# ethz-asl/laser_slam

Measured on AMD Instinct MI355X. Metric: scans_per_sec, higher is better.
Workload: dtype f32

## Files before the change

### laser_slam_amd/csrc/lsgpu_cone.hip.h

```cpp
#pragma once
#include "lsgpu_knn.hip.h"

namespace lsgpu {

constexpr int kConeGF4 = 3;
constexpr int kConePad = 16;
constexpr uint32_t kConeMaxWin = 512;

struct ConeDev {
  float ox, oy, oz;
  float z0, rs;
  float cs;
  int rows, cols;
  const float4* soa;
  const uint32_t* map;
  const uint32_t* tab;
  const float4* rowz;
};

__device__ __forceinline__ void cone_dir(float vx, float vy, float vz, float& inv_rho, float& zeta, float& pa, float& rxy,
                                         float& inv_h) {
  const float r2 = __fmaf_rn(vy, vy, vx * vx);
  inv_rho = __builtin_amdgcn_rsqf(__fmaf_rn(vz, vz, r2));
  rxy = __builtin_amdgcn_sqrtf(r2);
// ... 119 lines not shown
      const float4 X1 = p1[0], Y1 = p1[1], Z1 = p1[2];
      const f32x2 d0 = dist2_pair(q2x, q2y, q2z, f32x2{X.x, X.y}, f32x2{Y.x, Y.y}, f32x2{Z.x, Z.y});
      const f32x2 d1 = dist2_pair(q2x, q2y, q2z, f32x2{X.z, X.w}, f32x2{Y.z, Y.w}, f32x2{Z.z, Z.w});
      const f32x2 e0 = dist2_pair(q2x, q2y, q2z, f32x2{X1.x, X1.y}, f32x2{Y1.x, Y1.y}, f32x2{Z1.x, Z1.y});
      const f32x2 e1 = dist2_pair(q2x, q2y, q2z, f32x2{X1.z, X1.w}, f32x2{Y1.z, Y1.w}, f32x2{Z1.z, Z1.w});
      const float m4 = fminf(fminf(fminf(d0.x, d0.y), d1.x), d1.y);
      const float n4 = fminf(fminf(fminf(e0.x, e0.y), e1.x), e1.y);
      sec = __builtin_amdgcn_fmed3f(best, m4, sec);
      best = fminf(best, m4);
      sec = __builtin_amdgcn_fmed3f(best, n4, sec);
      best = fminf(best, n4);
    }
  }
}

#ifndef LSGPU_CONE_WAVES
#define LSGPU_CONE_WAVES 4
#endif
#ifndef LSGPU_CONE_OCC
#define LSGPU_CONE_OCC 8
#endif
constexpr int kConeRowSlots = 4;

struct ConeRec { float qx, qy, qz, ub, lbn; int id_in, j; uint32_t pad; };

__device__ __forceinline__ void cone_barrier_lds() {
  asm volatile("s_waitcnt lgkmcnt(0)\n\ts_barrier" ::: "memory");
}
__device__ __forceinline__ uint32_t wave_min_u32(uint32_t v) { return ~wave_max_u32(~v); }

template <int WAVES, bool PROBE = false>
__global__ __launch_bounds__(WAVES * 64, LSGPU_CONE_OCC) void k_knn_cone(KnnArgs a, ConeDev c) {
  __shared__ ConeRec rec[WAVES * 64];
  __shared__ unsigned long long ne_mask[16];
  __shared__ uint32_t wcount[WAVES], wbelow[WAVES];
  extern __shared__ float4 rowz_sh[];
  const int lane = threadIdx.x & 63, w = threadIdx.x >> 6;
#ifdef LSGPU_KNN_STATS
  const long long ts0 = clock64();
  const uint32_t wall0 = (uint32_t)wall_clock64();
  long long t_rows = 0, t_stage = 0, t_eval = 0;
  uint32_t n_chunks = 0, n_steps = 0, n_groups = 0, n_rowslots = 0;
#endif
  const uint32_t tile = blockIdx.x * (uint32_t)WAVES + (uint32_t)w;
  int j = (int)(tile * 64u) + lane;
  const bool act = j < a.nq;
  float4 rraw = make_float4(0.f, 0.f, 0.f, 0.f), mp = rraw;
// ... 60 lines not shown
  if (sel_on) {
    const uint32_t bits = __float_as_uint(ub);
    const unsigned long long below = __ballot(act && skip && bits < sel_lo);
    if (act && skip && bits >= sel_lo && bits - sel_lo < sel_span) sel_inside(bits);
    nbelow1 = (uint32_t)__popcll(below);
  }
#ifdef LSGPU_KNN_STATS
  const long long ts2 = clock64();
#endif
  const unsigned long long sm = __ballot(act && !skip);
  if (lane == 0) { wcount[w] = (uint32_t)__popcll(sm); wbelow[w] = nbelow1; }
  cone_barrier_lds();
  uint32_t before = 0, total = 0;
#pragma unroll
  for (int k = 0; k < WAVES; ++k) { const uint32_t n = wcount[k]; before += k < w ? n : 0u; total += n; }
  if (sel_on && threadIdx.x == 0) {
    uint32_t nb = 0u;
#pragma unroll
    for (int k = 0; k < WAVES; ++k) nb += wbelow[k];
    if (nb) atomicAdd(&a.sel_below[(blockIdx.x & (kSelBelowSlots - 1)) * kSelBelowStride], nb);
  }
  if (act && !skip) {
    ConeRec r;
    r.qx = qx; r.qy = qy; r.qz = qz; r.ub = ub; r.lbn = lbn; r.id_in = id_in; r.j = j; r.pad = 0u;
    const uint32_t at = before + (uint32_t)__popcll(sm & ((1ull << lane) - 1ull));
    rec[at] = r;
  }
  cone_barrier_lds();
#ifdef LSGPU_KNN_STATS
  const long long ts3 = clock64();
  if (lane == 0 && dbg) {
    dbg[0] = (uint32_t)(ts1 - ts0); dbg[1] = (uint32_t)(ts2 - ts1); dbg[2] = (uint32_t)(ts3 - ts2);
    dbg[3] = 1u; dbg[10] = (uint32_t)(ts3 - ts0); dbg[11] = wall0; dbg[12] = (uint32_t)wall_clock64();
    dbg[13] = (uint32_t)__popcll(sm);
  }
#endif
  if ((uint32_t)(w * 64) >= total) return;
  const bool ing = (uint32_t)(w * 64 + lane) < total;
  {
    const ConeRec r = rec[w * 64 + lane];
    qx = r.qx; qy = r.qy; qz = r.qz; ub = r.ub; lbn = r.lbn; id_in = r.id_in; j = r.j;
  }
  float inv_rho, zeta, pa, rxy, inv_h;
  cone_dir(qx - c.ox, qy - c.oy, qz - c.oz, inv_rho, zeta, pa, rxy, inv_h);
  float ubs = ub;
  if (PROBE) {
    const bool pr = ing && fabsf(zeta) <= 1.5f && pa >= 0.f && pa <= 4.f;
    const int rq = (int)cone_clampu(floorf((zeta - c.z0) * c.rs), c.rows - 1);
    const int cq = (int)cone_clampu(floorf(pa * c.cs), c.cols - 1);
    const uint32_t p_first = (uint32_t)__builtin_amdgcn_readfirstlane((int)wave_max_u32(pr ? ~(uint32_t)max(rq - 2, 0) : 0u));
    const uint32_t p_last = wave_max_u32(pr ? (uint32_t)min(rq + 2, c.rows - 1) + 1u : 0u);
    float pb = INFINITY, ps = INFINITY;
    for (uint32_t row = ~p_first; row < p_last; ++row) {
      const float4 rz = rowz_sh[row];
      if (!(rz.x <= rz.y)) continue;
      const bool in = pr && (int)row >= rq - 2 && (int)row <= rq + 2;
      const uint32_t base = row * (uint32_t)c.cols;
      uint32_t st_ = 0u, en_ = 0u;
      if (in) {
        st_ = c.tab[base + (uint32_t)max(cq - 1, 0)];
        en_ = c.tab[base + (uint32_t)min(cq + 1, c.cols - 1) + 1u];
      }
      const uint32_t g0 = st_ >> 2;
      const uint32_t len = en_ > st_ ? min(((en_ + 3u) >> 2) - g0, 4u) : 0u;
      cone_eval_window(c, g0, len, qx, qy, qz, pb, ps);
    }
    ubs = fminf(ub, pb);
  }
  const float lim0 = prune_lim(ubs, gap, cap2s);
  const float R = __builtin_amdgcn_sqrtf(lim0) * (1.0f + 1e-5f) + 1e-7f;
  bool fb = false;
  float best = INFINITY, sec = INFINITY, bs4 = INFINITY;
  float4 bpt = make_float4(0.f, 0.f, 0.f, 0.f);
  bool found = false;
  uint32_t bgrp = 0xFFFFFFFFu;
  {
    const float s = R * inv_rho * (1.0f + 1e-5f) + 4e-6f;
    const float ce = rxy * inv_rho;
    bool cone = ing && s <= 0.5f && ce > 0.f && ce <= 1.5f;
    const float alpha = s * (1.0f + 0.2f * s * s) + 2e-6f;
    const float alpha2 = alpha * alpha;
    const float dz = __fmaf_rn(ce, s, fabsf(zeta) * s * s) + 2e-6f;
    const float gq = (rxy * inv_h) * (rxy * inv_h) * (1.0f + 1e-6f);
    const float inv_ce = __builtin_amdgcn_rcpf(ce) * (1.0f + 1e-6f);
    const uint32_t r_lo = cone_clampu(floorf((zeta - dz - c.z0) * c.rs), c.rows - 1);
    const uint32_t r_hi = cone_clampu(floorf((zeta + dz - c.z0) * c.rs), c.rows - 1);
    fb = ing && !cone;
    const int cols = c.cols;
    const f32x2 q2x = {qx, qx}, q2y = {qy, qy}, q2z = {qz, qz};
    uint32_t row = (uint32_t)__builtin_amdgcn_readfirstlane((int)wave_min_u32(cone ? r_lo : 0xFFFFFFFFu));
    const uint32_t row_last = wave_max_u32(cone ? r_hi + 1u : 0u);
    int pass = 0;
    uint32_t n_st = 0u, n_en = 0u;
// ... 67 lines not shown
          const float4* __restrict__ p0 = c.soa + (uint32_t)kConeGF4 * (size_t)t;
          const float4* __restrict__ p1 = two ? p0 + kConeGF4 : p0;
          const float4 X = p0[0], Y = p0[1], Z = p0[2];
          const float4 X1 = p1[0], Y1 = p1[1], Z1 = p1[2];
          const f32x2 d0 = dist2_pair(q2x, q2y, q2z, f32x2{X.x, X.y}, f32x2{Y.x, Y.y}, f32x2{Z.x, Z.y});
          const f32x2 d1 = dist2_pair(q2x, q2y, q2z, f32x2{X.z, X.w}, f32x2{Y.z, Y.w}, f32x2{Z.z, Z.w});
          const f32x2 e0 = dist2_pair(q2x, q2y, q2z, f32x2{X1.x, X1.y}, f32x2{Y1.x, Y1.y}, f32x2{Z1.x, Z1.y});
          const f32x2 e1 = dist2_pair(q2x, q2y, q2z, f32x2{X1.z, X1.w}, f32x2{Y1.z, Y1.w}, f32x2{Z1.z, Z1.w});
          const float m4 = fminf(fminf(fminf(d0.x, d0.y), d1.x), d1.y);
          const float n4 = two ? fminf(fminf(fminf(e0.x, e0.y), e1.x), e1.y) : INFINITY;
          sec = __builtin_amdgcn_fmed3f(best, m4, sec);
          bgrp = m4 < best ? t : bgrp;
          best = fminf(best, m4);
          sec = __builtin_amdgcn_fmed3f(best, n4, sec);
          bgrp = n4 < best ? t + 1u : bgrp;
          best = fminf(best, n4);
        }
      }
#ifdef LSGPU_KNN_STATS
      t_eval += clock64() - t_s1;
#endif
    }
  }
  if (bgrp != 0xFFFFFFFFu) {
    const float4* __restrict__ p = c.soa + (uint32_t)kConeGF4 * (size_t)bgrp;
    const float4 X = p[0], Y = p[1], Z = p[2];
    const uint4 m = reinterpret_cast<const uint4*>(c.map)[bgrp];
    const float4 M = make_float4(__uint_as_float(m.x), __uint_as_float(m.y), __uint_as_float(m.z), __uint_as_float(m.w));
    const float e0 = dist2(qx - X.x, qy - Y.x, qz - Z.x), e1 = dist2(qx - X.y, qy - Y.y, qz - Z.y);
    const float e2 = dist2(qx - X.z, qy - Y.z, qz - Z.z), e3 = dist2(qx - X.w, qy - Y.w, qz - Z.w);
    if (e3 == best) bpt = make_float4(X.w, Y.w, Z.w, M.w);
    if (e2 == best) bpt = make_float4(X.z, Y.z, Z.z, M.z);
    if (e1 == best) bpt = make_float4(X.y, Y.y, Z.y, M.y);
    if (e0 == best) bpt = make_float4(X.x, Y.x, Z.x, M.x);
    bs4 = fminf(fmaxf(fminf(e0, e1), fminf(e2, e3)), fminf(fmaxf(e0, e1), fmaxf(e2, e3)));
    found = true;
  }
#ifdef LSGPU_KNN_STATS
  const long long ts5 = clock64();
#endif
  int bi = id_in;
  mp = make_float4(0.f, 0.f, 0.f, __int_as_float(id_in));
  const unsigned long long fbm = __ballot(fb);
  if (fbm) {
    if (fb) {
      best = ub;
      lane_ball_search(a, cap2s, qx, qy, qz, best, bi);
      if (bi != id_in) { const float4 p = a.pts[bi]; mp = make_float4(p.x, p.y, p.z, __int_as_float(bi)); }
    }
    if (lane == 0) atomicAdd(a.strag_count, (uint32_t)__popcll(fbm));
  }
  if (ing) {
    float nb;
    if (fb) {
      nb = best <= cap2s ? sqrtf(best) * (1.0f - 1e-6f) : fmaxf(lbn, sqrtf(cap2s) * (1.0f - 1e-5f));
    } else if (found && best <= ub) {
      mp = bpt;
      sec = fminf(sec, bs4);
      float others = fminf(sec, lim0);
      bool same = __float_as_int(mp.w) == id_in;
      if (sec == best || (!same && best == ub)) {
        mp = canonical_tie(a, qx, qy, qz, best, mp);
        same = __float_as_int(mp.w) == id_in;
      }
      if (!same) others = fminf(others, ub);
      nb = __builtin_amdgcn_sqrtf(others) * (1.0f - 1e-5f);
      if (same) nb = fmaxf(nb, lbn);
    } else {
      nb = fmaxf(__builtin_amdgcn_sqrtf(fminf(best, lim0)) * (1.0f - 1e-5f), lbn);
      best = ub;
    }
    if (a.write_all || __float_as_int(mp.w) != id_in) {
      a.ids[j] = __float_as_int(mp.w);
      a.prev[j] = mp;
    }
    a.d2[j] = best;
    a.lb[j] = nb;
  }
  if (sel_on) {
    const uint32_t bits = __float_as_uint(best);
    const unsigned long long below = __ballot(ing && bits < sel_lo);
    if (ing && bits >= sel_lo && bits - sel_lo < sel_span) sel_inside(bits);
    if (lane == 0 && below) atomicAdd(&a.sel_below[((tile + 32u) & (kSelBelowSlots - 1)) * kSelBelowStride], (uint32_t)__popcll(below));
  }
#ifdef LSGPU_KNN_STATS
  {
    const long long ts9 = clock64();
// ... 12 lines not shown
```

### laser_slam_amd/csrc/lsgpu_knn.hip.h

```cpp
#pragma once
#include "lsgpu_common.hip.h"

namespace lsgpu {

constexpr float kPruneShrink = 1.0f - 2e-6f;
constexpr float kCapSearchMargin2 = 1.05f * 1.05f;
constexpr float kPadCoord = 3e18f;

constexpr int kPriceSlots = 64, kPriceStride = 32;
struct ConePrice {
  float ox, oy, oz, rs, cs, dens4;
  float heavy;
  uint32_t* count;
};
__device__ __forceinline__ float cone_price(const ConePrice& c, float qx, float qy, float qz, float R) {
  const float vx = qx - c.ox, vy = qy - c.oy, vz = qz - c.oz;
  const float r2 = __fmaf_rn(vy, vy, vx * vx);
  const float inv_rho = __builtin_amdgcn_rsqf(__fmaf_rn(vz, vz, r2));
  const float rxy = __builtin_amdgcn_sqrtf(r2);
  const float sn = R * inv_rho, ce = rxy * inv_rho, zeta = fabsf(vz * inv_rho);
  const float g = rxy * __builtin_amdgcn_rcpf(fabsf(vx) + fabsf(vy));
  const float rows = 2.f * (ce * sn + zeta * sn * sn) * c.rs + 1.f;
  const float cols = 2.f * (g * g) * sn * __builtin_amdgcn_rcpf(ce) * c.cs + 1.f;
  const bool served = sn <= 0.5f && ce > 0.05f && ce <= 1.5f;
// ... 92 lines not shown
      continue;
    const uint32_t p0 = a.chunks[cs].start;
    const ChunkDesc dl = a.chunks[l == 0 ? ce - 1 : cs];
    uint32_t p1 = dl.start + dl.count;
    if (p1 - p0 > 256u) p1 = p0 + 256u;
    float best = INFINITY;
    for (uint32_t t = p0; t < p1; t += 4) {
      const float4 c0 = a.pts[t], c1 = a.pts[t + 1], c2 = a.pts[t + 2], c3 = a.pts[t + 3];
      const float d0 = dist2(q.x - c0.x, q.y - c0.y, q.z - c0.z), d1 = dist2(q.x - c1.x, q.y - c1.y, q.z - c1.z);
      const float d2 = dist2(q.x - c2.x, q.y - c2.y, q.z - c2.z), d3 = dist2(q.x - c3.x, q.y - c3.y, q.z - c3.z);
      if (d0 < best) { best = d0; bi = (int)t; bp = c0; }
      if (d1 < best) { best = d1; bi = (int)t + 1; bp = c1; }
      if (d2 < best) { best = d2; bi = (int)t + 2; bp = c2; }
      if (d3 < best) { best = d3; bi = (int)t + 3; bp = c3; }
    }
    bd = best;
    break;
  }
  a.prev[j] = make_float4(bp.x, bp.y, bp.z, __int_as_float(bi));
  a.d2[j] = bd;
  if (a.lb) a.lb[j] = 0.f;
}

__device__ __forceinline__ void lane_ball_search(const KnnArgs& a, float cap2, float qx, float qy, float qz,
                                                 float& best, int& bi) {
  const GridDev& g = a.g;
  float prune = fminf(best, cap2);
  const float R = sqrtf(prune) * (1.0f + 1e-5f) + 1e-7f + kFineSlack * g.hf;
  const int lim = (1 << (g.bits + g.fine)) - 1;
  const int flx = fine_coord(qx - R, g.ox, g.inv_hf, lim), fhx = fine_coord(qx + R, g.ox, g.inv_hf, lim);
  const int fly = fine_coord(qy - R, g.oy, g.inv_hf, lim), fhy = fine_coord(qy + R, g.oy, g.inv_hf, lim);
  const int flz = fine_coord(qz - R, g.oz, g.inv_hf, lim), fhz = fine_coord(qz + R, g.oz, g.inv_hf, lim);
  int l = 0, sh = g.fine;
  for (; l < g.bits; ++l, ++sh)
    if ((fhx >> sh) - (flx >> sh) < 2 && (fhy >> sh) - (fly >> sh) < 2 && (fhz >> sh) - (flz >> sh) < 2)
      break;
  sh = g.fine + l;
  const int x0 = flx >> sh, y0 = fly >> sh, z0 = flz >> sh;
  const int x1 = fhx >> sh, y1 = fhy >> sh, z1 = fhz >> sh;
  const uint32_t mask = g.mask[l];
  const uint4* tab = reinterpret_cast<const uint4*>(g.tab[l]);
  uint4 en[8];
  uint32_t slot[8];
  bool want[8];
#pragma unroll
  for (int c = 0; c < 8; ++c) {
    const int cx = x0 + (c & 1), cy = y0 + ((c >> 1) & 1), cz = z0 + (c >> 2);
    want[c] = cx <= x1 && cy <= y1 && cz <= z1;
    slot[c] = cell_hash((uint32_t)cx, (uint32_t)cy, (uint32_t)cz) & mask;
    en[c] = make_uint4(kEmpty, 0u, 0u, 0u);
    if (want[c]) en[c] = tab[slot[c]];
  }
#pragma unroll
  for (int c = 0; c < 8; ++c) {
    if (!want[c]) continue;
    const uint32_t cx = (uint32_t)(x0 + (c & 1)), cy = (uint32_t)(y0 + ((c >> 1) & 1)), cz = (uint32_t)(z0 + (c >> 2));
    const uint32_t xy = cx | (cy << 16);
    uint4 e = en[c];
    uint32_t sl = slot[c];
    while (!(((e.x ^ xy) | (e.y ^ cz)) == 0u) && e.x != kEmpty) {
      sl = (sl + 1) & mask;
      e = tab[sl];
    }
    if (e.x == kEmpty) continue;
    for (uint32_t ch = e.z; ch < e.w; ++ch) {
      if ((ch & (uint32_t)(kChunkGroup - 1)) == 0u && ch + (uint32_t)kChunkGroup <= e.w) {
        const float4* gd = reinterpret_cast<const float4*>(a.cgroups + ch / (uint32_t)kChunkGroup);
        const float4 g0 = gd[0], g1 = gd[1];
        if (!(box_dist2(g0.x, g0.y, g0.z, g1.x, g1.y, g1.z, qx, qy, qz) * kPruneShrink <= prune)) { ch += (uint32_t)kChunkGroup - 1u; continue; }
      }
      const float4* cd = reinterpret_cast<const float4*>(a.chunks + ch);
      const float4 b0 = cd[0], b1 = cd[1];
      if (!(box_dist2(b0.x, b0.y, b0.z, b1.x, b1.y, b1.z, qx, qy, qz) * kPruneShrink <= prune)) continue;
      const uint32_t st = __float_as_uint(b0.w), cnt = __float_as_uint(b1.w);
      for (uint32_t t = 0; t < cnt; t += 4) {
        const float4 p0 = a.pts[st + t], p1 = a.pts[st + t + 1], p2 = a.pts[st + t + 2], p3 = a.pts[st + t + 3];
        const float d0 = dist2(qx - p0.x, qy - p0.y, qz - p0.z);
        const float d1 = dist2(qx - p1.x, qy - p1.y, qz - p1.z);
        const float d2 = dist2(qx - p2.x, qy - p2.y, qz - p2.z);
        const float d3 = dist2(qx - p3.x, qy - p3.y, qz - p3.z);
        if (d0 < best || (d0 == best && (int)(st + t) < bi)) { best = d0; bi = (int)(st + t); }
        if (d1 < best || (d1 == best && (int)(st + t + 1) < bi)) { best = d1; bi = (int)(st + t + 1); }
        if (d2 < best || (d2 == best && (int)(st + t + 2) < bi)) { best = d2; bi = (int)(st + t + 2); }
        if (d3 < best || (d3 == best && (int)(st + t + 3) < bi)) { best = d3; bi = (int)(st + t + 3); }
      }
      prune = fminf(best, cap2);
    }
  }
}

__device__ __forceinline__ float4 canonical_tie(const KnnArgs& a, float qx, float qy, float qz, float best, float4 mp) {
  int bi = __float_as_int(mp.w);
  const int before = bi;
  float b = best;
  lane_ball_search(a, INFINITY, qx, qy, qz, b, bi);
  if (bi != before) { const float4 p = a.pts[bi]; mp = make_float4(p.x, p.y, p.z, __int_as_float(bi)); }
  return mp;
}

constexpr int kListCap = 128;
constexpr uint32_t kChunkBudget = 1024;

struct TileLds {
  float4 slot[4][64];
  uint32_t list[kListCap];
};

typedef float f32x2 __attribute__((ext_vector_type(2)));

__device__ __forceinline__ f32x2 dist2_pair(f32x2 qx, f32x2 qy, f32x2 qz, f32x2 cx, f32x2 cy, f32x2 cz) {
  const f32x2 dx = qx - cx, dy = qy - cy, dz = qz - cz;
  f32x2 d = dx * dx;
  d = __builtin_elementwise_fma(dy, dy, d);
  d = __builtin_elementwise_fma(dz, dz, d);
  return d;
}

__device__ __forceinline__ float prune_lim(float b, float gap, float cap2) {
  return fminf(__fmaf_rn(2.f * gap, __builtin_amdgcn_sqrtf(b), b) + gap * gap, cap2);
}

__device__ __forceinline__ void tile_eval_slot(const float4* __restrict__ slot, uint32_t st, uint32_t cnt,
                                               float qx, float qy, float qz, float& best, float& sec, int& grp) {
  const uint32_t c4 = (cnt + 3u) >> 2;
  const f32x2 q2x = {qx, qx}, q2y = {qy, qy}, q2z = {qz, qz};
#pragma unroll 2
  for (uint32_t t = 0; t < c4; ++t) {
    const float4 x = slot[t], y = slot[c4 + t], z = slot[2u * c4 + t];
// ... 180 lines not shown
    na += issue(1, sa1, ca1);
    if (na == 2) asm volatile("s_waitcnt vmcnt(2)" ::: "memory");
    else if (na == 1) asm volatile("s_waitcnt vmcnt(1)" ::: "memory");
    else asm volatile("s_waitcnt vmcnt(0)" ::: "memory");
    n_eval += nb;
    if (SPLIT && sp.ways > 1) {
      tile_eval_slot_split(lds.slot[2], sb0, cb0, lane, sp);
      if (nb > 1) tile_eval_slot_split(lds.slot[3], sb1, cb1, lane, sp);
    } else {
      tile_eval_slot(lds.slot[2], sb0, cb0, qx, qy, qz, best, sec, grp);
      if (nb > 1) tile_eval_slot(lds.slot[3], sb1, cb1, qx, qy, qz, best, sec, grp);
    }
  }
  if (SPLIT && sp.ways > 1) split_merge(sp, ing, __ballot(ing), lane, best, sec, grp);
  maxbest = wave_max(ing ? prune_lim(fminf(best, ub), gap, cap2) : 0.f);
#ifdef LSGPU_KNN_STATS
  c_eval += (uint32_t)(clock64() - t_ev0);
#else
  (void)c_eval;
#endif
}

__device__ __forceinline__ float4 tile_resolve_match(const KnnArgs& a, int grp, float qx, float qy, float qz,
                                                     float best, float4 mp, float& s4) {
  if (grp >= 0) {
    const float4 p0 = a.pts[grp], p1 = a.pts[grp + 1], p2 = a.pts[grp + 2], p3 = a.pts[grp + 3];
    const float e0 = dist2(qx - p0.x, qy - p0.y, qz - p0.z), e1 = dist2(qx - p1.x, qy - p1.y, qz - p1.z);
    const float e2 = dist2(qx - p2.x, qy - p2.y, qz - p2.z), e3 = dist2(qx - p3.x, qy - p3.y, qz - p3.z);
    if (e3 == best) mp = make_float4(p3.x, p3.y, p3.z, __int_as_float(grp + 3));
    if (e2 == best) mp = make_float4(p2.x, p2.y, p2.z, __int_as_float(grp + 2));
    if (e1 == best) mp = make_float4(p1.x, p1.y, p1.z, __int_as_float(grp + 1));
    if (e0 == best) mp = make_float4(p0.x, p0.y, p0.z, __int_as_float(grp));
    s4 = fminf(fmaxf(fminf(e0, e1), fminf(e2, e3)), fminf(fmaxf(e0, e1), fmaxf(e2, e3)));
  }
  return mp;
}

constexpr int kRowqList = 64;

__device__ __forceinline__ void rowq_search(const KnnArgs& a, float cap2s, float gap, uint32_t* list, int row, int k16,
                                            bool have, float qx, float qy, float qz, float ub, int id_in,
                                            unsigned long long& bestp_out, float& sec_out) {
  const GridDev& g = a.g;
  const int lim = (1 << (g.bits + g.fine)) - 1;
  unsigned long long bestp = have ? (((unsigned long long)__float_as_uint(ub) << 32) | (uint32_t)id_in) : ~0ull;
  float bcur = ub;
  float sec = INFINITY;
  float best = prune_lim(bcur, gap, cap2s);
  uint32_t cs = 0, ce = 0;
  {
    const float B = sqrtf(best) * (1.0f + 1e-5f) + 1e-7f + kFineSlack * g.hf;
    const int flx = fine_coord(qx - B, g.ox, g.inv_hf, lim), fhx = fine_coord(qx + B, g.ox, g.inv_hf, lim);
    const int fly = fine_coord(qy - B, g.oy, g.inv_hf, lim), fhy = fine_coord(qy + B, g.oy, g.inv_hf, lim);
    const int flz = fine_coord(qz - B, g.oz, g.inv_hf, lim), fhz = fine_coord(qz + B, g.oz, g.inv_hf, lim);
    int l = 0;
// ... 174 lines not shown
#ifndef LSGPU_TILE_OCC_SPLIT
#define LSGPU_TILE_OCC_SPLIT 6
#endif
template <int WAVES, bool LAZY = false, bool SPLIT = false>
__global__ __launch_bounds__(WAVES * 64, SPLIT ? LSGPU_TILE_OCC_SPLIT : LSGPU_TILE_OCC) void k_knn_tile(KnnArgs a) {
  static_assert(!(LAZY && SPLIT), "the lazy instantiation re-tests chunks against bounds the parts have not merged yet");
  __shared__ TileLds lds_all[WAVES];
  const int lane = threadIdx.x & 63, w = threadIdx.x >> 6;
  TileLds& lds = lds_all[w];
#ifdef LSGPU_KNN_STATS
  const long long t_begin = clock64();
#endif
  const uint32_t wpb = blockDim.x >> 6;
  uint32_t blk = blockIdx.x;
  if (WAVES == 1 && a.front_blocks > 0) {
    if (blk < (uint32_t)a.front_blocks) {
      tile_front_rows(a, reinterpret_cast<uint32_t*>(lds.slot), lane, blk);
      return;
    }
    blk -= (uint32_t)a.front_blocks;
  }
  const uint32_t tile = blk * wpb + w;
  if (tile >= (uint32_t)a.ntiles) return;
  const int j = (int)(tile * 64u) + lane;
  const bool act = j < a.nq;
  float4 rraw = make_float4(0.f, 0.f, 0.f, 0.f), mp = rraw;
  float lb_in = 0.f;
  if (act) {
    rraw = a.rdq[j];
    mp = a.prev[j];
    if (a.lb) lb_in = a.lb[j];
  }
  const int id_in = __float_as_int(mp.w);
  const uint32_t on_list = a.spread_flag ? a.spread_flag[tile] : 0u;
  if (on_list && a.front_blocks > 0) {
    const uint32_t covered = min(a.spread_cnt[0], (uint32_t)a.front_blocks / (uint32_t)kFrontPerTile);
    if (on_list - 1u < covered) return;
  }
  ulonglong2 tag_pre = make_ulonglong2(0ull, 0ull);
  uint2 cc_pre = make_uint2(0u, 0u);
  if (a.cell_cache) {
    tag_pre = a.cell_tags[tile];
    cc_pre = a.cell_cache[(size_t)tile * 64 + lane];
  }
  Mat34 T; float cap2;
  if (!iter_params(a.st, a.T, a.cap2, a.use_state_cap, T, cap2)) return;
  const float cap2s = cap2 * kCapSearchMargin2;
#ifdef LSGPU_KNN_STATS
  if ((a.dbg_flags & 1024) && (tile & 1u)) return;
  if ((a.dbg_flags & 2048) && (tile & 3u)) return;
#endif
  const GridDev& g = a.g;
  uint32_t n_eval = 0, n_surv = 0, n_grp = 0, lvl_max = 0, c_eval = 0;

  float qx = 0.f, qy = 0.f, qz = 0.f, ub = 0.f, best = INFINITY, sec = INFINITY;
  int bi = -1, grp = -1;
  if (act) {
    const float3 q = xform(T, rraw.x, rraw.y, rraw.z);
    qx = q.x; qy = q.y; qz = q.z;
    bi = __float_as_int(mp.w);
    ub = dist2(qx - mp.x, qy - mp.y, qz - mp.z);
  }
#ifdef LSGPU_KNN_STATS
  asm volatile("s_waitcnt vmcnt(0)" ::: "memory");
  const long long t_loaded = clock64();
  long long t_red = t_loaded, t_look = t_loaded;
#endif
  float lbn = 0.f;
  bool skip = false;
  const float gap = a.use_state_cap ? a.gap : 0.f;
  if (act && a.lb && a.st && a.use_state_cap) {
    Mat34 To;
#pragma unroll
    for (int i = 0; i < 12; ++i) To.m[i] = a.st->T_rows_prev[i];
    const float3 qo = xform(To, rraw.x, rraw.y, rraw.z);
    const float ddx = qx - qo.x, ddy = qy - qo.y, ddz = qz - qo.z;
    const float delta = sqrtf(ddx * ddx + ddy * ddy + ddz * ddz) * (1.0f + 1e-5f) + 1e-7f;
    lbn = fmaxf(lb_in * (1.0f - 1e-6f) - delta, 0.f);
    const float lb2 = lbn * lbn;
    const bool keep = ub * (1.0f + 1e-5f) < lb2;
    const bool far = fminf(ub, lb2) > cap2 * (1.0f + 1e-5f);
    skip = keep || far;
  }
  const float R = sqrtf(prune_lim(ub, gap, cap2s)) * (1.0f + 1e-5f) + 1e-7f;
  const bool straggler = act && !skip && !(R <= a.r_cap);
  const bool ing = act && !straggler && !skip;
  bool routed = false;
  const unsigned long long ing_mask = __ballot(ing);
  if (a.price.count) {
    const unsigned long long hv = __ballot(ing && !(cone_price(a.price, qx, qy, qz, R) <= a.price.heavy));
    if (lane == 0 && ing_mask) {
      uint32_t* slot = a.price.count + (tile & (uint32_t)(kPriceSlots - 1)) * (uint32_t)kPriceStride;
      if (hv) atomicAdd(slot, (uint32_t)__popcll(hv));
      atomicAdd(slot + 1, (uint32_t)__popcll(ing_mask));
    }
  }
#ifdef LSGPU_KNN_STATS
  if (ing_mask && !(a.dbg_flags & 4)) {
#else
  if (ing_mask) {
#endif
    const float tlx = wave_min(ing ? qx : INFINITY), thx = wave_max(ing ? qx : -INFINITY);
    const float tly = wave_min(ing ? qy : INFINITY), thy = wave_max(ing ? qy : -INFINITY);
    const float tlz = wave_min(ing ? qz : INFINITY), thz = wave_max(ing ? qz : -INFINITY);
    const float Rmax = wave_max(ing ? R : 0.f);
    float maxbest = wave_max(ing ? prune_lim(ub, gap, cap2s) : 0.f);
    const int lim = (1 << (g.bits + g.fine)) - 1;
    const float pad = Rmax + kFineSlack * g.hf;
    const int flx = __builtin_amdgcn_readfirstlane(fine_coord(tlx - pad, g.ox, g.inv_hf, lim));
    const int fly = __builtin_amdgcn_readfirstlane(fine_coord(tly - pad, g.oy, g.inv_hf, lim));
    const int flz = __builtin_amdgcn_readfirstlane(fine_coord(tlz - pad, g.oz, g.inv_hf, lim));
    const int fhx = __builtin_amdgcn_readfirstlane(fine_coord(thx + pad, g.ox, g.inv_hf, lim));
    const int fhy = __builtin_amdgcn_readfirstlane(fine_coord(thy + pad, g.oy, g.inv_hf, lim));
    const int fhz = __builtin_amdgcn_readfirstlane(fine_coord(thz + pad, g.oz, g.inv_hf, lim));
#ifdef LSGPU_KNN_STATS
    t_red = clock64();
#endif
    int l = 0, sh = g.fine;
    for (; l < g.bits; ++l, ++sh)
      if ((fhx >> sh) - (flx >> sh) < 4 && (fhy >> sh) - (fly >> sh) < 4 && (fhz >> sh) - (flz >> sh) < 4)
        break;
    sh = g.fine + l;
    const int x0 = flx >> sh, y0 = fly >> sh, z0 = flz >> sh;
    const int nx = (fhx >> sh) - x0 + 1, ny = (fhy >> sh) - y0 + 1, nz = (fhz >> sh) - z0 + 1;
#ifdef LSGPU_KNN_STATS
    if (a.dbg_flags & 512) { if (lane == 0 && nx + ny + nz == -7) a.d2[0] = 0.f; return; }
#endif
// ... 22 lines not shown
    asm volatile("s_waitcnt vmcnt(0)" ::: "memory");
    t_look = clock64();
#endif
    const float ext = fmaxf(fmaxf(thx - tlx, thy - tly), thz - tlz);
    const uint32_t block_chunks = wave_sum_u32(ce - cs);
    const bool spread = ext > fmaxf(a.group_r, 4.f * Rmax) && block_chunks > (uint32_t)a.chunk_budget;
    if (spread && a.spread_list && !on_list && lane == 0) {
      const uint32_t idx = atomicAdd(&a.spread_cnt[1], 1u);
      if (idx < (uint32_t)kFrontMax) { a.spread_list[idx] = tile; a.spread_flag[tile] = idx + 1u; }
    }
    bool heavy = Rmax > a.spread_route_r && !spread && block_chunks > (uint32_t)a.route_chunks;
    if (a.spread_route_r > 0.f && heavy && a.route_heavy_max >= 0) {
      uint32_t t = 0u;
      if (lane == 0) t = atomicAdd(a.strag_count + 2, 1u);
      heavy = (uint32_t)__builtin_amdgcn_readfirstlane((int)t) < (uint32_t)a.route_heavy_max;
    }
#ifdef LSGPU_KNN_STATS
    if (spread && (a.dbg_flags & 32)) {  } else
#endif
    if (a.spread_route_r > 0.f && (heavy || (spread && (Rmax > a.spread_route_r || block_chunks > (uint32_t)a.route_dense)))) {
      routed = ing;
    } else if (spread) {
      if (ing) {
        const int before = bi;
        best = ub;
        lane_ball_search(a, cap2s, qx, qy, qz, best, bi);
        if (bi != before) { const float4 p = a.pts[bi]; mp = make_float4(p.x, p.y, p.z, __int_as_float(bi)); }
      }
      n_grp = 64;
    } else {
      n_grp = 1; lvl_max = l;
#ifdef LSGPU_KNN_STATS
      if (a.dbg_flags & 64) return;
#endif
      SplitState sp;
      sp.ways = 1;
      if (SPLIT) split_setup(sp, ing_mask, lane, qx, qy, qz);
      if (LAZY && block_chunks > (uint32_t)a.route_chunks) sp.ways = -1;
      unsigned long long cells = __ballot(ce > cs);
      uint32_t fill = 0;
      while (cells) {
        const int c = __ffsll((long long)cells) - 1;
        cells &= cells - 1;
        const uint32_t ccs = rl_u(cs, c), cce = rl_u(ce, c);
        for (uint32_t base = ccs; base < cce; base += 64) {
          const uint32_t n = (cce - base) < 64u ? (cce - base) : 64u;
          if ((uint32_t)lane < n) lds.list[fill + lane] = base + lane;
          fill += n;
          while (fill >= 64u) {
            fill -= 64u;
            const uint32_t ch = lds.list[fill + lane];
            tile_process_batch<LAZY, SPLIT>(a, cap2s, lds, lane, true, ch, ing, qx, qy, qz, tlx, tly, tlz, thx, thy, thz,
                               maxbest, ub, gap, best, sec, grp, n_eval, n_surv, c_eval, sp);
          }
        }
      }
      if (fill) {
        const bool v = (uint32_t)lane < fill;
        const uint32_t ch = v ? lds.list[lane] : 0u;
        tile_process_batch<LAZY, SPLIT>(a, cap2s, lds, lane, v, ch, ing, qx, qy, qz, tlx, tly, tlz, thx, thy, thz,
                           maxbest, ub, gap, best, sec, grp, n_eval, n_surv, c_eval, sp);
      }
    }
  }
#ifdef LSGPU_KNN_STATS
  if (a.dbg_flags & (64 | 128 | 256 | 512)) return;
  const long long t_loop_end = clock64();
#endif
  if (act) {
    float nb;
    if (routed) {
      best = ub;
      nb = lbn;
    } else if (n_grp == 64 && ing) {
      nb = best <= cap2s ? sqrtf(best) * (1.0f - 1e-6f) : fmaxf(lbn, sqrtf(cap2s) * (1.0f - 1e-5f));
    } else if (!ing) {
      best = ub;
      nb = lbn;
    } else {
      const float lim_f = prune_lim(fminf(best, ub), gap, cap2s);
      if (best <= ub) {
        float s4 = INFINITY;
        mp = tile_resolve_match(a, grp, qx, qy, qz, best, mp, s4);
        float others = fminf(fminf(sec, s4), lim_f);
        bool same = __float_as_int(mp.w) == bi;
        if (sec == best || (!same && best == ub)) {
          mp = canonical_tie(a, qx, qy, qz, best, mp);
          same = __float_as_int(mp.w) == bi;
        }
        if (!same) others = fminf(others, ub);
        nb = sqrtf(others) * (1.0f - 1e-5f);
        if (same) nb = fmaxf(nb, lbn);
      } else {
        nb = fmaxf(sqrtf(fminf(best, lim_f)) * (1.0f - 1e-5f), lbn);
        best = ub;
      }
    }
    if (a.write_all || __float_as_int(mp.w) != id_in) {
      a.ids[j] = __float_as_int(mp.w);
      a.prev[j] = mp;
    }
    a.d2[j] = best;
    if (a.lb) a.lb[j] = nb;
  }
  {
    const unsigned long long hm = __ballot(act && (straggler || routed));
    if (hm) {
      uint32_t base = 0;
      if (lane == 0) base = atomicAdd(a.strag_count, (uint32_t)__popcll(hm));
      base = (uint32_t)__builtin_amdgcn_readfirstlane((int)base);
      if (act && (straggler || routed)) a.strag[base + (uint32_t)__popcll(hm & ((1ull << lane) - 1ull))] = (uint32_t)j;
    }
  }
  if (a.sel_below && (a.st->sel_mode || a.sel_force)) {
    const bool fin = act && !routed && !straggler;
    const uint32_t bits = __float_as_uint(best), lo = a.st->sel_lo;
    const unsigned long long below = __ballot(fin && bits < lo);
    if (fin && bits >= lo && bits - lo < a.st->sel_span) sel_count_inside(a, bits);
    if (lane == 0 && below) atomicAdd(&a.sel_below[(tile & (kSelBelowSlots - 1)) * kSelBelowStride], (uint32_t)__popcll(below));
  }
#ifdef LSGPU_KNN_STATS
  const uint32_t n_act = (uint32_t)__popcll(__ballot(ing));
  if (lane == 0 && a.dbg) {
    atomicAdd(&a.dbg[1], (unsigned long long)(t_loaded - t_begin)); atomicAdd(&a.dbg[2], (unsigned long long)(t_red - t_loaded));
// ... 123 lines not shown
```

Baseline: 251.8.

## Spill live state to LDS and restructure ball search to cut register pressure

The cone and tile kNN kernels now keep values that live across the search loops (lbn, id_in, j, lim0) in LDS records and reload them afterwards, instead of holding them in VGPRs. The fallback ball search is moved ahead of match resolution, and tie canonicalisation is wave-gated. lane_ball_search is rewritten with explicit per-cell probes and resolves plus a non-unrolled select loop. The tile kernel also recomputes j and cap2s from uniform values and skips rewriting prev when the point is unchanged. The intent is lower VGPR use and higher occupancy, at the cost of extra LDS traffic and subtle changes to the write-back semantics; a register-usage diff tool is added.

```diff
diff --git a/devtools/kernel_resources.py b/devtools/kernel_resources.py
--- /dev/null
+++ b/devtools/kernel_resources.py
@@ -0,0 +1,101 @@
+#!/usr/bin/env python3
+import os
+import re
+import subprocess
+import sys
+
+FIELDS = (("vgpr", ".vgpr_count"), ("agpr", ".agpr_count"), ("sgpr", ".sgpr_count"),
+          ("private", ".private_segment_fixed_size"), ("lds", ".group_segment_fixed_size"))
+READELF = os.environ.get("LLVM_READELF", "/opt/rocm/llvm/bin/llvm-readelf")
+
+
+def metadata_lines(path):
+    with open(path, "rb") as f:
+        elf = f.read(4) == b"\x7fELF"
+    if elf:
+        return subprocess.run([READELF, "--notes", path], capture_output=True, text=True, check=True).stdout.split("\n")
+    out, inside = [], False
+    for line in open(path, errors="replace"):
+        if line.startswith("\t.amdgpu_metadata") or line.startswith(".amdgpu_metadata"):
+            inside = True
+        elif line.lstrip().startswith(".end_amdgpu_metadata"):
+            inside = False
+        elif inside:
+            out.append(line.rstrip("\n"))
+    return out
+
+
+def strip_arguments(name):
+    if not name.endswith(")"):
+        return name
+    depth = 0
+    for i in range(len(name) - 1, -1, -1):
+        depth += name[i] == ")"
+        depth -= name[i] == "("
+        if depth == 0:
+            return name[:i]
+    return name
+
+
+def kernels(path):
+    res, cur = [], None
+    for line in metadata_lines(path):
+        m = re.match(r"\s*(- )?(\.[a-z_]+):\s*(.*)$", line)
+        if not m:
+            continue
+        if m.group(1) and re.match(r"\s{0,4}- ", line):
+            cur = {}
+            res.append(cur)
+        if cur is None:
+            continue
+        key, val = m.group(2), m.group(3).strip().strip("'\"")
+        if key == ".name" and not re.match(r"\s{6,}", line):
+            cur["name"] = val
+        for short, field in FIELDS:
+            if key == field:
+                cur[short] = int(val, 0)
+    named = [k for k in res if "name" in k and "vgpr" in k]
+    dem = subprocess.run(["c++filt"], input="\n".join(k["name"] for k in named), capture_output=True, text=True).stdout.split("\n")
+    out = {}
+    for k, d in zip(named, dem):
+        d = re.sub(r"^void ", "", d)
+        d = strip_arguments(d).replace("lsgpu::", "")
+        out[d] = {s: k.get(s, 0) for s, _ in FIELDS}
+    return out
+
+
+def row(name, k):
+    return f"{name:<84} {k['vgpr']:>5} {k['agpr']:>5} {k['sgpr']:>5} {k['private']:>8} {k['lds']:>7}"
+
+
+def main():
+    head = f"{'kernel':<84} {'vgpr':>5} {'agpr':>5} {'sgpr':>5} {'private':>8} {'lds':>7}"
+    if len(sys.argv) == 2:
+        ks = kernels(sys.argv[1])
+        print(head)
+        for n in sorted(ks):
+            print(row(n, ks[n]))
+        print(f"{len(ks)} kernels, {sum(1 for k in ks.values() if k['private'])} with a private segment")
+        return 0
+    if len(sys.argv) != 3:
+        print(__doc__)
+        return 2
+    a, b = kernels(sys.argv[1]), kernels(sys.argv[2])
+    print("  " + head + "      (<: first, >: second, >!: more VGPRs or a larger private segment)")
+    worse = 0
+    for n in sorted(set(a) & set(b)):
+        if a[n] != b[n]:
+            up = b[n]["vgpr"] > a[n]["vgpr"] or b[n]["private"] > a[n]["private"]
+            worse += up
+            print("< " + row(n, a[n]))
+            print(("> " if not up else ">!") + row(n, b[n]))
+    for n in sorted(set(b) - set(a)):
+        print("+ " + row(n, b[n]))
+    for n in sorted(set(a) - set(b)):
+        print("- " + row(n, a[n]))
+    print(f"{len(set(a) & set(b))} kernels in both, {worse} with more VGPRs or a larger private segment in the second")
+    return 1 if worse else 0
+
+
+if __name__ == "__main__":
+    sys.exit(main())
diff --git a/laser_slam_amd/csrc/lsgpu_cone.hip.h b/laser_slam_amd/csrc/lsgpu_cone.hip.h
--- a/laser_slam_amd/csrc/lsgpu_cone.hip.h
+++ b/laser_slam_amd/csrc/lsgpu_cone.hip.h
@@ -165,7 +165,10 @@
 #endif
 constexpr int kConeRowSlots = 4;
 
-struct ConeRec { float qx, qy, qz, ub, lbn; int id_in, j; uint32_t pad; };
+struct ConeRec {
+  float qx, qy, qz, ub, lbn; int id_in, j;
+  float lim0;
+};
 
 __device__ __forceinline__ void cone_barrier_lds() {
   asm volatile("s_waitcnt lgkmcnt(0)\n\ts_barrier" ::: "memory");
@@ -272,7 +275,7 @@
   }
   if (act && !skip) {
     ConeRec r;
-    r.qx = qx; r.qy = qy; r.qz = qz; r.ub = ub; r.lbn = lbn; r.id_in = id_in; r.j = j; r.pad = 0u;
+    r.qx = qx; r.qy = qy; r.qz = qz; r.ub = ub; r.lbn = lbn; r.id_in = id_in; r.j = j; r.lim0 = 0.f;
     const uint32_t at = before + (uint32_t)__popcll(sm & ((1ull << lane) - 1ull));
     rec[at] = r;
   }
@@ -288,8 +291,8 @@
   if ((uint32_t)(w * 64) >= total) return;
   const bool ing = (uint32_t)(w * 64 + lane) < total;
   {
-    const ConeRec r = rec[w * 64 + lane];
-    qx = r.qx; qy = r.qy; qz = r.qz; ub = r.ub; lbn = r.lbn; id_in = r.id_in; j = r.j;
+    const ConeRec& r = rec[w * 64 + lane];
+    qx = r.qx; qy = r.qy; qz = r.qz; ub = r.ub;
   }
   float inv_rho, zeta, pa, rxy, inv_h;
   cone_dir(qx - c.ox, qy - c.oy, qz - c.oz, inv_rho, zeta, pa, rxy, inv_h);
@@ -317,8 +320,9 @@
     }
     ubs = fminf(ub, pb);
   }
-  const float lim0 = prune_lim(ubs, gap, cap2s);
+  float lim0 = prune_lim(ubs, gap, cap2s);
   const float R = __builtin_amdgcn_sqrtf(lim0) * (1.0f + 1e-5f) + 1e-7f;
+  rec[w * 64 + lane].lim0 = lim0;
   bool fb = false;
   float best = INFINITY, sec = INFINITY, bs4 = INFINITY;
   float4 bpt = make_float4(0.f, 0.f, 0.f, 0.f);
@@ -432,7 +436,19 @@
 #endif
     }
   }
-  if (bgrp != 0xFFFFFFFFu) {
+  const ConeRec& myrec = rec[w * 64 + lane];
+  int bi = 0;
+  const unsigned long long fbm = __ballot(fb);
+  if (fbm) {
+    if (fb) {
+      bi = myrec.id_in;
+      best = ub;
+      lane_ball_search(a, cap2s, qx, qy, qz, best, bi);
+    }
+    if (lane == 0) atomicAdd(a.strag_count, (uint32_t)__popcll(fbm));
+    asm volatile("" ::: "memory");
+  }
+  if (bgrp != 0xFFFFFFFFu && !fb) {
     const float4* __restrict__ p = c.soa + (uint32_t)kConeGF4 * (size_t)bgrp;
     const float4 X = p[0], Y = p[1], Z = p[2];
     const uint4 m = reinterpret_cast<const uint4*>(c.map)[bgrp];
@@ -449,30 +465,26 @@
 #ifdef LSGPU_KNN_STATS
   const long long ts5 = clock64();
 #endif
-  int bi = id_in;
+  lbn = myrec.lbn; id_in = myrec.id_in; j = myrec.j; lim0 = myrec.lim0;
   mp = make_float4(0.f, 0.f, 0.f, __int_as_float(id_in));
-  const unsigned long long fbm = __ballot(fb);
-  if (fbm) {
-    if (fb) {
-      best = ub;
-      lane_ball_search(a, cap2s, qx, qy, qz, best, bi);
-      if (bi != id_in) { const float4 p = a.pts[bi]; mp = make_float4(p.x, p.y, p.z, __int_as_float(bi)); }
-    }
-    if (lane == 0) atomicAdd(a.strag_count, (uint32_t)__popcll(fbm));
+  if (fb && bi != id_in) { const float4 p = a.pts[bi]; mp = make_float4(p.x, p.y, p.z, __int_as_float(bi)); }
+  const bool hit = ing && !fb && found && best <= ub;
+  if (hit) { mp = bpt; sec = fminf(sec, bs4); }
+  {
+    const bool tie = hit && (sec == best || (__float_as_int(mp.w) != id_in && best == ub));
+    if (__ballot(tie)) {
+      if (tie) mp = canonical_tie(a, qx, qy, qz, best, mp);
+      asm volatile("" ::: "memory");
+      lbn = myrec.lbn; id_in = myrec.id_in; j = myrec.j; lim0 = myrec.lim0;
+    }
   }
   if (ing) {
     float nb;
     if (fb) {
       nb = best <= cap2s ? sqrtf(best) * (1.0f - 1e-6f) : fmaxf(lbn, sqrtf(cap2s) * (1.0f - 1e-5f));
-    } else if (found && best <= ub) {
-      mp = bpt;
-      sec = fminf(sec, bs4);
+    } else if (hit) {
       float others = fminf(sec, lim0);
-      bool same = __float_as_int(mp.w) == id_in;
-      if (sec == best || (!same && best == ub)) {
-        mp = canonical_tie(a, qx, qy, qz, best, mp);
-        same = __float_as_int(mp.w) == id_in;
-      }
+      const bool same = __float_as_int(mp.w) == id_in;
       if (!same) others = fminf(others, ub);
       nb = __builtin_amdgcn_sqrtf(others) * (1.0f - 1e-5f);
       if (same) nb = fmaxf(nb, lbn);
diff --git a/laser_slam_amd/csrc/lsgpu_knn.hip.h b/laser_slam_amd/csrc/lsgpu_knn.hip.h
--- a/laser_slam_amd/csrc/lsgpu_knn.hip.h
+++ b/laser_slam_amd/csrc/lsgpu_knn.hip.h
@@ -138,6 +138,33 @@
   if (a.lb) a.lb[j] = 0.f;
 }
 
+__device__ __forceinline__ uint4 ball_probe(const uint4* __restrict__ tab, uint32_t mask, int cx, int cy, int cz, bool want) {
+  uint4 e = make_uint4(kEmpty, 0u, 0u, 0u);
+  if (want) e = tab[cell_hash((uint32_t)cx, (uint32_t)cy, (uint32_t)cz) & mask];
+  return e;
+}
+__device__ __forceinline__ void ball_resolve(const uint4* __restrict__ tab, uint32_t mask, uint4 e, int cx_, int cy_, int cz_,
+                                             uint32_t& cb, uint32_t& ce) {
+  const uint32_t cx = (uint32_t)cx_, cy = (uint32_t)cy_, cz = (uint32_t)cz_;
+  const uint32_t xy = cx | (cy << 16);
+  if (!(((e.x ^ xy) | (e.y ^ cz)) == 0u) && e.x != kEmpty) {
+    uint32_t sl = cell_hash(cx, cy, cz) & mask;
+    do {
+      sl = (sl + 1) & mask;
+      e = tab[sl];
+    } while (!(((e.x ^ xy) | (e.y ^ cz)) == 0u) && e.x != kEmpty);
+  }
+  const bool hit = e.x != kEmpty;
+  cb = hit ? e.z : 0u;
+  ce = hit ? e.w : 0u;
+}
+__device__ __forceinline__ uint32_t ball_sel8(int c, uint32_t v0, uint32_t v1, uint32_t v2, uint32_t v3, uint32_t v4,
+                                              uint32_t v5, uint32_t v6, uint32_t v7) {
+  const uint32_t a0 = c & 1 ? v1 : v0, a1 = c & 1 ? v3 : v2, a2 = c & 1 ? v5 : v4, a3 = c & 1 ? v7 : v6;
+  const uint32_t b0 = c & 2 ? a1 : a0, b1 = c & 2 ? a3 : a2;
+  return c & 4 ? b1 : b0;
+}
+
 __device__ __forceinline__ void lane_ball_search(const KnnArgs& a, float cap2, float qx, float qy, float qz,
                                                  float& best, int& bi) {
   const GridDev& g = a.g;
@@ -155,32 +182,30 @@
   const int x0 = flx >> sh, y0 = fly >> sh, z0 = flz >> sh;
   const int x1 = fhx >> sh, y1 = fhy >> sh, z1 = fhz >> sh;
   const uint32_t mask = g.mask[l];
-  const uint4* tab = reinterpret_cast<const uint4*>(g.tab[l]);
-  uint4 en[8];
-  uint32_t slot[8];
-  bool want[8];
-#pragma unroll
+  const uint4* __restrict__ tab = reinterpret_cast<const uint4*>(g.tab[l]);
+  const bool wx = x0 + 1 <= x1, wy = y0 + 1 <= y1, wz = z0 + 1 <= z1;
+  const uint4 e0 = ball_probe(tab, mask, x0, y0, z0, true);
+  const uint4 e1 = ball_probe(tab, mask, x0 + 1, y0, z0, wx);
+  const uint4 e2 = ball_probe(tab, mask, x0, y0 + 1, z0, wy);
+  const uint4 e3 = ball_probe(tab, mask, x0 + 1, y0 + 1, z0, wx && wy);
+  const uint4 e4 = ball_probe(tab, mask, x0, y0, z0 + 1, wz);
+  const uint4 e5 = ball_probe(tab, mask, x0 + 1, y0, z0 + 1, wx && wz);
+  const uint4 e6 = ball_probe(tab, mask, x0, y0 + 1, z0 + 1, wy && wz);
+  const uint4 e7 = ball_probe(tab, mask, x0 + 1, y0 + 1, z0 + 1, wx && wy && wz);
+  uint32_t cb0, cb1, cb2, cb3, cb4, cb5, cb6, cb7, ce0, ce1, ce2, ce3, ce4, ce5, ce6, ce7;
+  ball_resolve(tab, mask, e0, x0, y0, z0, cb0, ce0);
+  ball_resolve(tab, mask, e1, x0 + 1, y0, z0, cb1, ce1);
+  ball_resolve(tab, mask, e2, x0, y0 + 1, z0, cb2, ce2);
+  ball_resolve(tab, mask, e3, x0 + 1, y0 + 1, z0, cb3, ce3);
+  ball_resolve(tab, mask, e4, x0, y0, z0 + 1, cb4, ce4);
+  ball_resolve(tab, mask, e5, x0 + 1, y0, z0 + 1, cb5, ce5);
+  ball_resolve(tab, mask, e6, x0, y0 + 1, z0 + 1, cb6, ce6);
+  ball_resolve(tab, mask, e7, x0 + 1, y0 + 1, z0 + 1, cb7, ce7);
+#pragma nounroll
   for (int c = 0; c < 8; ++c) {
-    const int cx = x0 + (c & 1), cy = y0 + ((c >> 1) & 1), cz = z0 + (c >> 2);
-    want[c] = cx <= x1 && cy <= y1 && cz <= z1;
-    slot[c] = cell_hash((uint32_t)cx, (uint32_t)cy, (uint32_t)cz) & mask;
-    en[c] = make_uint4(kEmpty, 0u, 0u, 0u);
-    if (want[c]) en[c] = tab[slot[c]];
-  }
-#pragma unroll
-  for (int c = 0; c < 8; ++c) {
-    if (!want[c]) continue;
-    const uint32_t cx = (uint32_t)(x0 + (c & 1)), cy = (uint32_t)(y0 + ((c >> 1) & 1)), cz = (uint32_t)(z0 + (c >> 2));
-    const uint32_t xy = cx | (cy << 16);
-    uint4 e = en[c];
-    uint32_t sl = slot[c];
-    while (!(((e.x ^ xy) | (e.y ^ cz)) == 0u) && e.x != kEmpty) {
-      sl = (sl + 1) & mask;
-      e = tab[sl];
-    }
-    if (e.x == kEmpty) continue;
-    for (uint32_t ch = e.z; ch < e.w; ++ch) {
-      if ((ch & (uint32_t)(kChunkGroup - 1)) == 0u && ch + (uint32_t)kChunkGroup <= e.w) {
+    const uint32_t ch_end = ball_sel8(c, ce0, ce1, ce2, ce3, ce4, ce5, ce6, ce7);
+    for (uint32_t ch = ball_sel8(c, cb0, cb1, cb2, cb3, cb4, cb5, cb6, cb7); ch < ch_end; ++ch) {
+      if ((ch & (uint32_t)(kChunkGroup - 1)) == 0u && ch + (uint32_t)kChunkGroup <= ch_end) {
         const float4* gd = reinterpret_cast<const float4*>(a.cgroups + ch / (uint32_t)kChunkGroup);
         const float4 g0 = gd[0], g1 = gd[1];
         if (!(box_dist2(g0.x, g0.y, g0.z, g1.x, g1.y, g1.z, qx, qy, qz) * kPruneShrink <= prune)) { ch += (uint32_t)kChunkGroup - 1u; continue; }
@@ -214,12 +239,16 @@
   return mp;
 }
 
+__device__ __forceinline__ float uni_f(float v) {
+  return __int_as_float(__builtin_amdgcn_readfirstlane(__float_as_int(v)));
+}
 constexpr int kListCap = 128;
 constexpr uint32_t kChunkBudget = 1024;
 
 struct TileLds {
   float4 slot[4][64];
   uint32_t list[kListCap];
+  int id_in[64];
 };
 
 typedef float f32x2 __attribute__((ext_vector_type(2)));
@@ -446,7 +475,7 @@
 }
 
 __device__ __forceinline__ float4 tile_resolve_match(const KnnArgs& a, int grp, float qx, float qy, float qz,
-                                                     float best, float4 mp, float& s4) {
+                                                     float best, float4 mp, float& s4, bool& repl) {
   if (grp >= 0) {
     const float4 p0 = a.pts[grp], p1 = a.pts[grp + 1], p2 = a.pts[grp + 2], p3 = a.pts[grp + 3];
     const float e0 = dist2(qx - p0.x, qy - p0.y, qz - p0.z), e1 = dist2(qx - p1.x, qy - p1.y, qz - p1.z);
@@ -455,6 +484,7 @@
     if (e2 == best) mp = make_float4(p2.x, p2.y, p2.z, __int_as_float(grp + 2));
     if (e1 == best) mp = make_float4(p1.x, p1.y, p1.z, __int_as_float(grp + 1));
     if (e0 == best) mp = make_float4(p0.x, p0.y, p0.z, __int_as_float(grp));
+    repl = repl || e0 == best || e1 == best || e2 == best || e3 == best;
     s4 = fminf(fmaxf(fminf(e0, e1), fminf(e2, e3)), fminf(fmaxf(e0, e1), fmaxf(e2, e3)));
   }
   return mp;
@@ -675,16 +705,16 @@
   }
   const uint32_t tile = blk * wpb + w;
   if (tile >= (uint32_t)a.ntiles) return;
-  const int j = (int)(tile * 64u) + lane;
-  const bool act = j < a.nq;
+  const int j0 = (int)(tile * 64u) + lane;
+  const bool act = j0 < a.nq;
   float4 rraw = make_float4(0.f, 0.f, 0.f, 0.f), mp = rraw;
   float lb_in = 0.f;
   if (act) {
-    rraw = a.rdq[j];
-    mp = a.prev[j];
-    if (a.lb) lb_in = a.lb[j];
-  }
-  const int id_in = __float_as_int(mp.w);
+    rraw = a.rdq[j0];
+    mp = a.prev[j0];
+    if (a.lb) lb_in = a.lb[j0];
+  }
+  lds.id_in[lane] = __float_as_int(mp.w);
   const uint32_t on_list = a.spread_flag ? a.spread_flag[tile] : 0u;
   if (on_list && a.front_blocks > 0) {
     const uint32_t covered = min(a.spread_cnt[0], (uint32_t)a.front_blocks / (uint32_t)kFrontPerTile);
@@ -707,13 +737,14 @@
   uint32_t n_eval = 0, n_surv = 0, n_grp = 0, lvl_max = 0, c_eval = 0;
 
   float qx = 0.f, qy = 0.f, qz = 0.f, ub = 0.f, best = INFINITY, sec = INFINITY;
-  int bi = -1, grp = -1;
+  int grp = -1;
   if (act) {
     const float3 q = xform(T, rraw.x, rraw.y, rraw.z);
     qx = q.x; qy = q.y; qz = q.z;
-    bi = __float_as_int(mp.w);
     ub = dist2(qx - mp.x, qy - mp.y, qz - mp.z);
   }
+  mp = make_float4(0.f, 0.f, 0.f, mp.w);
+  bool repl = false;
 #ifdef LSGPU_KNN_STATS
   asm volatile("s_waitcnt vmcnt(0)" ::: "memory");
   const long long t_loaded = clock64();
@@ -753,9 +784,9 @@
 #else
   if (ing_mask) {
 #endif
-    const float tlx = wave_min(ing ? qx : INFINITY), thx = wave_max(ing ? qx : -INFINITY);
-    const float tly = wave_min(ing ? qy : INFINITY), thy = wave_max(ing ? qy : -INFINITY);
-    const float tlz = wave_min(ing ? qz : INFINITY), thz = wave_max(ing ? qz : -INFINITY);
+    const float tlx = uni_f(wave_min(ing ? qx : INFINITY)), thx = uni_f(wave_max(ing ? qx : -INFINITY));
+    const float tly = uni_f(wave_min(ing ? qy : INFINITY)), thy = uni_f(wave_max(ing ? qy : -INFINITY));
+    const float tlz = uni_f(wave_min(ing ? qz : INFINITY)), thz = uni_f(wave_max(ing ? qz : -INFINITY));
     const float Rmax = wave_max(ing ? R : 0.f);
     float maxbest = wave_max(ing ? prune_lim(ub, gap, cap2s) : 0.f);
     const int lim = (1 << (g.bits + g.fine)) - 1;
@@ -824,10 +855,11 @@
       routed = ing;
     } else if (spread) {
       if (ing) {
-        const int before = bi;
+        const int before = lds.id_in[lane];
+        int bi = before;
         best = ub;
         lane_ball_search(a, cap2s, qx, qy, qz, best, bi);
-        if (bi != before) { const float4 p = a.pts[bi]; mp = make_float4(p.x, p.y, p.z, __int_as_float(bi)); }
+        if (bi != before) { const float4 p = a.pts[bi]; mp = make_float4(p.x, p.y, p.z, __int_as_float(bi)); repl = true; }
       }
       n_grp = 64;
     } else {
@@ -869,26 +901,30 @@
   if (a.dbg_flags & (64 | 128 | 256 | 512)) return;
   const long long t_loop_end = clock64();
 #endif
+  asm volatile("" ::: "memory");
+  const int id_in = lds.id_in[lane];
+  const int j = (int)((uint32_t)__builtin_amdgcn_readfirstlane((int)tile) * 64u) + lane;
+  const float cap2s_e = __int_as_float(__builtin_amdgcn_readfirstlane(__float_as_int(cap2))) * kCapSearchMargin2;
   if (act) {
     float nb;
     if (routed) {
       best = ub;
       nb = lbn;
     } else if (n_grp == 64 && ing) {
-      nb = best <= cap2s ? sqrtf(best) * (1.0f - 1e-6f) : fmaxf(lbn, sqrtf(cap2s) * (1.0f - 1e-5f));
+      nb = best <= cap2s_e ? sqrtf(best) * (1.0f - 1e-6f) : fmaxf(lbn, sqrtf(cap2s_e) * (1.0f - 1e-5f));
     } else if (!ing) {
       best = ub;
       nb = lbn;
     } else {
-      const float lim_f = prune_lim(fminf(best, ub), gap, cap2s);
+      const float lim_f = prune_lim(fminf(best, ub), gap, cap2s_e);
       if (best <= ub) {
         float s4 = INFINITY;
-        mp = tile_resolve_match(a, grp, qx, qy, qz, best, mp, s4);
+        mp = tile_resolve_match(a, grp, qx, qy, qz, best, mp, s4, repl);
         float others = fminf(fminf(sec, s4), lim_f);
-        bool same = __float_as_int(mp.w) == bi;
+        bool same = __float_as_int(mp.w) == id_in;
         if (sec == best || (!same && best == ub)) {
           mp = canonical_tie(a, qx, qy, qz, best, mp);
-          same = __float_as_int(mp.w) == bi;
+          same = __float_as_int(mp.w) == id_in;
         }
         if (!same) others = fminf(others, ub);
         nb = sqrtf(others) * (1.0f - 1e-5f);
@@ -898,10 +934,9 @@
         best = ub;
       }
     }
-    if (a.write_all || __float_as_int(mp.w) != id_in) {
-      a.ids[j] = __float_as_int(mp.w);
-      a.prev[j] = mp;
-    }
+    const bool changed = __float_as_int(mp.w) != id_in;
+    if (a.write_all || changed) a.ids[j] = __float_as_int(mp.w);
+    if (changed || (a.write_all && repl)) a.prev[j] = mp;
     a.d2[j] = best;
     if (a.lb) a.lb[j] = nb;
   }
```

Measured after the change: 255.1 (median of 6 runs). About the same (+1.3%).
